# r9y9/deepvoice3_pytorch

Measured on NVIDIA H100. Metric: mel-frames/sec training step (B=16,T_mel=800), higher is better.
Workload: dtype f32 via split 16-bit pairs (fp16 pairs forward, bf16 pairs for gradients; 3 wgmma passes per product, fp32 accumulate)

## Files before the change

deepvoice3_pytorch_b200/csrc/tc_gemm.cu:

```cuda
#include "tc_common.cuh"
#include "../../include/dv3b200.h"

namespace dv3 {

using namespace tc;

constexpr int TC_CONV_THREADS = 512;
constexpr int TC_PRODUCER_REGS = 24;
constexpr int TC_CONSUMER_REGS = 176;
constexpr int TC_EPILOGUE_REGS = 136;
static_assert(TC_PRODUCER_REGS <= 65536 / TC_CONV_THREADS && TC_CONSUMER_REGS >= 65536 / TC_CONV_THREADS &&
              TC_EPILOGUE_REGS >= 65536 / TC_CONV_THREADS, "setmaxnreg direction of each warpgroup");
static_assert(128 * TC_PRODUCER_REGS + 256 * TC_CONSUMER_REGS + 128 * TC_EPILOGUE_REGS <= 65536, "register file");
constexpr int MAX_TAPS_TC = 8;
constexpr int SMEM_LIMIT = 232448;
constexpr int RING_RESERVE = 32768;

template <int STAGE_BYTES, int TILE_COLS, int RESERVE>
struct RingCfg {
    static constexpr int STAGE = STAGE_BYTES;
    static constexpr int NCOLS = TILE_COLS;
    static constexpr int ACC_PITCH = NCOLS + 1;
    static constexpr int ACC_TILE = 128 * ACC_PITCH * 4;
    static constexpr int STAGES_RAW = (SMEM_LIMIT - 2048 - RESERVE - ACC_TILE) / STAGE;
    static constexpr int STAGES = STAGES_RAW > 6 ? 6 : STAGES_RAW;
    static constexpr int SMEM = STAGES * STAGE + ACC_TILE + 1024 + 512;
};

enum { TC_GATED = 0, TC_CONV = 1 };

struct TcMaps { CUtensorMap a[2]; CUtensorMap b[2]; };

struct TcParams {
    int T;
    int Nc;
    int rows_per_tap;
    int k, kb_n;
    int tap_off[MAX_TAPS_TC];
    const float* bias; const float* spk; const float* res;
    float* y; float* save_a; float* save_s;
    int gate_mode, residual;
    float* out; const float* e1; const float* e2; float alpha; int addmode, relu;
    float p_drop; const unsigned long long* seed_ptr; uint32_t salt;
    float gmain;
    int operand_bf16;
};

template <int BK> struct SwizzleOf;
template <> struct SwizzleOf<64> { static constexpr uint32_t layout = WG_SW128, sbo = 1024; };
template <> struct SwizzleOf<32> { static constexpr uint32_t layout = WG_SW64, sbo = 512; };

template <int BK>
__device__ __forceinline__ uint64_t make_desc(uint32_t saddr) {
    return make_wgmma_desc(saddr, 16, SwizzleOf<BK>::sbo, SwizzleOf<BK>::layout);
}

template <int NBOX, int BK, int BR, int NPL = 2>
using TcCfg = RingCfg<NPL * (128 + NBOX * BR) * BK * 2, BR * NBOX, RING_RESERVE>;
static_assert(TcCfg<2, 32, 64>::STAGES == 4, "gated forward: 4-stage ring");
static_assert(TcCfg<1, 32, 128>::STAGES == 4, "128-column conv: 4-stage ring");
static_assert(TcCfg<1, 64, 64>::STAGES == 3, "64-column conv at BK = 64: 3-stage ring");
static_assert(TcCfg<1, 32, 64>::STAGES == 6, "64-column conv at BK = 32: 6-stage ring");
static_assert(TcCfg<2, 64, 64, 1>::STAGES == 4, "single-pass gated forward: 4-stage ring");
static_assert(TcCfg<1, 64, 128, 1>::STAGES == 4, "single-pass 128-column conv at BK = 64: 4-stage ring");
static_assert(TcCfg<1, 32, 128, 1>::STAGES == 6, "single-pass 128-column conv at BK = 32: 6-stage ring");
static_assert(TcCfg<1, 64, 64, 1>::STAGES == 6, "single-pass 64-column conv at BK = 64: 6-stage ring");
static_assert(TcCfg<1, 32, 64, 1>::STAGES == 6, "single-pass 64-column conv at BK = 32: 6-stage ring");

template <int BR>
__device__ __forceinline__ void epilogue_gated(const TcParams& p, const float* arow, uint64_t* acc_empty, int a_row0,
                                               int a_z, int b_row0) {
    const int t = a_row0 + (threadIdx.x & 127), b = a_z, C = p.Nc;
    const bool tv = t < p.T;
    const float* __restrict__ bias = p.bias;
    const float* __restrict__ res = p.res;
    const float* __restrict__ spk = p.spk;
    float* __restrict__ yo = p.y;
    float* __restrict__ ao = p.save_a;
    float* __restrict__ so = p.save_s;
    const bool need_res = (p.gate_mode != 0) || p.residual;
    const size_t base = ((size_t)b * C + b_row0) * p.T + (tv ? t : 0);
#pragma unroll
    for (int c32 = 0; c32 < BR; c32 += 32) {
        float rr[32], sp[32];
        if (tv) {
            const size_t cb = base + (size_t)c32 * p.T;
#pragma unroll
            for (int i = 0; i < 32; ++i) rr[i] = need_res ? __ldg(&res[cb + (size_t)i * p.T]) : 0.f;
            if (spk) {
#pragma unroll
                for (int i = 0; i < 32; ++i) sp[i] = __ldg(&spk[cb + (size_t)i * p.T]);
            }
#pragma unroll
            for (int i = 0; i < 32; ++i) {
                const int c = b_row0 + c32 + i;
                const size_t idx = cb + (size_t)i * p.T;
                float va = arow[c32 + i];
                if (spk) va += sp[i];
                const float a = va + __ldg(&bias[c]);
                const float s = sigmoidf_(arow[BR + c32 + i] + __ldg(&bias[C + c]));
                float y;
                if (p.gate_mode == 0) {
                    y = a * s;
                    if (p.residual) y = (y + rr[i]) * 0.70710678118654752f;
                } else {
                    y = s * a + (1.f - s) * rr[i];
                }
                yo[idx] = y;
                if (ao) ao[idx] = a;
                if (so) so[idx] = s;
            }
        }
        if (c32 + 32 == BR) mbar_arrive(acc_empty);
    }
}

template <int NCOLS>
__device__ __forceinline__ void epilogue_conv(const TcParams& p, const float* arow, uint64_t* acc_empty, int a_row0,
                                              int a_z, int b_row0) {
    const int t = a_row0 + (threadIdx.x & 127), b = a_z;
    const bool tv = t < p.T;
    const DropCfg drop = make_drop(p.p_drop, p.seed_ptr, p.salt);
    const float* __restrict__ bias = p.bias;
    const float* __restrict__ e1 = p.e1;
    const float* __restrict__ e2 = p.e2;
    float* __restrict__ out = p.out;
#pragma unroll 1
    for (int c32 = 0; c32 < NCOLS; c32 += 32) {
        float v[32], x2[32];
        const int n0 = b_row0 + c32;
        const size_t cb = ((size_t)b * p.Nc + n0) * p.T + (tv ? t : 0);
        if (tv) {
#pragma unroll
            for (int i = 0; i < 32; ++i) {
                const bool ok = n0 + i < p.Nc;
                v[i] = (p.addmode != 0 && ok) ? __ldg(&e1[cb + (size_t)i * p.T]) : 0.f;
                x2[i] = (p.addmode == 2 && ok) ? __ldg(&e2[cb + (size_t)i * p.T]) : 0.f;
            }
#pragma unroll
            for (int i = 0; i < 32; ++i) {
                const int n = n0 + i;
                if (n < p.Nc) {
                    const size_t idx = cb + (size_t)i * p.T;
                    float g = arow[c32 + i] * drop_scale(drop, (uint32_t)idx);
                    if (bias) g += __ldg(&bias[n]);
                    if (p.addmode == 1) g += p.alpha * v[i];
                    else if (p.addmode == 2) g += v[i] * (1.f - x2[i]);
                    if (p.relu) g = fmaxf(g, 0.f);
                    out[idx] = g;
                }
            }
        }
        if (c32 + 32 == NCOLS) mbar_arrive(acc_empty);
    }
}

template <class Cfg, int NPL, class Decode, class Load, class Mma, class Gmain, class Epilogue>
__device__ __forceinline__ void tc_pipeline(const TcMaps& maps, int num_units, Decode decode, Load load, Mma mma,
                                            Gmain gmain, Epilogue epilogue) {
    static_assert(NPL == 1 || NPL == 2, "one or two operand planes");
    static_assert(Cfg::NCOLS <= 128, "main + cross accumulators must fit in the registers of a consumer thread");
    static_assert(Cfg::STAGES >= 2, "pipeline needs at least two stages");
    constexpr int STAGE = Cfg::STAGE, STAGES = Cfg::STAGES;
    constexpr int NR = Cfg::NCOLS / 2;
    pdl_trigger();
    extern __shared__ uint8_t smem_raw[];
    uint8_t* smem = reinterpret_cast<uint8_t*>((reinterpret_cast<uintptr_t>(smem_raw) + 1023) & ~(uintptr_t)1023);
    float* acc_tile = reinterpret_cast<float*>(smem + STAGES * STAGE);
    uint64_t* full = reinterpret_cast<uint64_t*>(smem + STAGES * STAGE + Cfg::ACC_TILE);
    uint64_t* empty = full + STAGES;
    uint64_t* acc_full = empty + STAGES;
    uint64_t* acc_empty = acc_full + 1;
    const int warp = threadIdx.x >> 5, lane = threadIdx.x & 31;

    if (threadIdx.x == 0) {
#pragma unroll
        for (int pl = 0; pl < NPL; ++pl) prefetch_tmap(&maps.a[pl]);
#pragma unroll
        for (int pl = 0; pl < NPL; ++pl) prefetch_tmap(&maps.b[pl]);
        for (int s = 0; s < STAGES; ++s) { mbar_init(&full[s], 1); mbar_init(&empty[s], 2); }
        mbar_init(acc_full, 256);
        mbar_init(acc_empty, 128);
        fence_barrier_init();
    }
    __syncthreads();
    pdl_wait();

    if (warp >= 12) {
        setmaxnreg_inc<TC_EPILOGUE_REGS>();
        int n = 0;
        for (int u = blockIdx.x; u < num_units; u += gridDim.x, ++n) {
            const auto w = decode(u);
            mbar_wait(acc_full, n & 1);
            epilogue(w, acc_tile, acc_empty);
        }
    } else if (warp >= 8) {
        setmaxnreg_dec<TC_PRODUCER_REGS>();
        if (warp == 8 && lane == 0) {
            int it = 0;
            for (int u = blockIdx.x; u < num_units; u += gridDim.x) {
                const auto w = decode(u);
                for (int kit = 0; kit < w.n_iters; ++kit, ++it) {
                    const int s = it % STAGES, ph = (it / STAGES) & 1;
                    mbar_wait(&empty[s], ph ^ 1);
                    mbar_arrive_expect_tx(&full[s], STAGE);
                    load(w, kit, smem + s * STAGE, &full[s]);
                }
            }
        }
    } else {
        setmaxnreg_inc<TC_CONSUMER_REGS>();
        const int wg = warp >> 2, wq = warp & 3;
        float acc[NR], xacc[NPL == 2 ? NR : 1];
        int it = 0, n = 0;
        for (int u = blockIdx.x; u < num_units; u += gridDim.x, ++n) {
            const auto w = decode(u);
#pragma unroll
            for (int i = 0; i < NR; ++i) {
                acc[i] = 0.f;
                if constexpr (NPL == 2) xacc[i] = 0.f;
            }
            for (int kit = 0; kit < w.n_iters; ++kit, ++it) {
                const int s = it % STAGES, ph = (it / STAGES) & 1;
                mbar_wait(&full[s], ph);
                wgmma_fence();
                mma(smem + s * STAGE, wg, acc, xacc);
                wgmma_commit();
                wgmma_wait<1>();
                if (kit > 0 && (threadIdx.x & 127) == 0) mbar_arrive(&empty[(it - 1) % STAGES]);
            }
            wgmma_wait<0>();
            if (w.n_iters > 0 && (threadIdx.x & 127) == 0) mbar_arrive(&empty[(it - 1) % STAGES]);
            const float gm = gmain(w);
            mbar_wait(acc_empty, (n & 1) ^ 1);
#pragma unroll
            for (int i = 0; i < NR; ++i) {
                float* dst = &acc_tile[(64 * wg + frag_row(i, wq, lane)) * Cfg::ACC_PITCH + frag_col(i, lane)];
                if constexpr (NPL == 2) *dst = fmaf(xacc[i], LO_INV, acc[i] * gm);
                else *dst = acc[i] * gm;
            }
            mbar_arrive(acc_full);
        }
    }
}

template <int MODE, int NBOX, int BR, int BK, bool BF16, int NPL>
__global__ void __launch_bounds__(TC_CONV_THREADS, 1)
tc_conv_kernel(const __grid_constant__ TcMaps maps, const __grid_constant__ TcParams p, int tiles_x, int tiles_y,
               int num_tiles) {
    using Cfg = TcCfg<NBOX, BK, BR, NPL>;
    constexpr int NCOLS = Cfg::NCOLS;
    constexpr int TILE = 128 * BK * 2, TILE_B = BR * BK * 2;
    constexpr int B_OFF = NPL * TILE;
    constexpr int A_HALF = 64 * BK * 2;
    const int n_iters = p.k * p.kb_n;

    struct Tile { int a_row0, a_z, b_row0, b_row1, n_iters; };
    auto decode = [&](int tile) {
        Tile w;
        const int ty = tile % tiles_y, r = tile / tiles_y;
        w.a_z = r / tiles_x;
        w.a_row0 = (r % tiles_x) * 128;
        if (MODE == TC_GATED) { w.b_row0 = ty * BR; w.b_row1 = p.Nc + ty * BR; }
        else { w.b_row0 = ty * BR * NBOX; w.b_row1 = w.b_row0 + BR; }
        w.n_iters = n_iters;
        return w;
    };
    auto load = [&](const Tile& w, int kit, uint8_t* st, uint64_t* bar) {
        const int j = kit / p.kb_n, kb = kit - j * p.kb_n;
        const int ax = kb * BK, ay = w.a_row0 + p.tap_off[j];
        const int by0 = j * p.rows_per_tap + w.b_row0, by1 = j * p.rows_per_tap + w.b_row1;
#pragma unroll
        for (int pl = 0; pl < NPL; ++pl) {
            tma_load_3d(st + pl * TILE, &maps.a[pl], bar, ax, ay, w.a_z);
            uint8_t* bdst = st + B_OFF + pl * NBOX * TILE_B;
            tma_load_3d(bdst, &maps.b[pl], bar, ax, by0, 0);
            if (NBOX == 2) tma_load_3d(bdst + TILE_B, &maps.b[pl], bar, ax, by1, 0);
        }
    };
    auto mma = [&](const uint8_t* st, int wg, float* acc, float* xacc) {
        const uint32_t sa = smem_u32(st) + wg * A_HALF, sb = smem_u32(st + B_OFF);
#pragma unroll
        for (int kk = 0; kk < BK / 16; ++kk) {
            const uint32_t ko = kk * 32;
            const uint64_t a0 = make_desc<BK>(sa + ko), b0 = make_desc<BK>(sb + ko);
            wgmma_mma<NCOLS, 0, 0>(BF16, acc, a0, b0, 1);
            if constexpr (NPL == 2) {
                const uint64_t a1 = make_desc<BK>(sa + TILE + ko), b1 = make_desc<BK>(sb + NBOX * TILE_B + ko);
                wgmma_mma<NCOLS, 0, 0>(BF16, xacc, a0, b1, 1);
                wgmma_mma<NCOLS, 0, 0>(BF16, xacc, a1, b0, 1);
            }
        }
    };
    auto gmain = [&](const Tile&) { return p.gmain; };
    auto epilogue = [&](const Tile& w, const float* acc_tile, uint64_t* acc_empty) {
        const float* arow = acc_tile + (threadIdx.x & 127) * Cfg::ACC_PITCH;
        if (MODE == TC_GATED) epilogue_gated<BR>(p, arow, acc_empty, w.a_row0, w.a_z, w.b_row0);
        else epilogue_conv<NCOLS>(p, arow, acc_empty, w.a_row0, w.a_z, w.b_row0);
    };
    tc_pipeline<Cfg, NPL>(maps, num_tiles, decode, load, mma, gmain, epilogue);
}

struct TcMnParams {
    int T, B, Mw, Nw, k;
    int tap_off[MAX_TAPS_TC];
    int nsplit, batches_per_split, kb_n;
    int tiles_n, tiles_m, num_units;
    float* dw; long long split_stride;
    int msplit; long long s_m, s_mh, s_n, s_j;
    float gcoef;
};

constexpr int WG_BOX = 64 * 32 * 2;
template <int NPL>
using WgCfg = RingCfg<NPL * 4 * WG_BOX, 128, 0>;
static_assert(WgCfg<2>::STAGES == 5, "two-plane weight gradient: 5-stage ring");
static_assert(WgCfg<1>::STAGES == 6, "single-pass weight gradient: 6-stage ring");
static_assert(WgCfg<2>::SMEM <= SMEM_LIMIT && WgCfg<1>::SMEM <= SMEM_LIMIT, "weight gradient shared memory");

template <int NPL>
__global__ void __launch_bounds__(TC_CONV_THREADS, 1)
tc_wgrad_mn_kernel(const __grid_constant__ TcMaps maps, const __grid_constant__ TcMnParams p) {
    using Cfg = WgCfg<NPL>;
    constexpr int A_PL = 2 * WG_BOX, B_PL = 2 * WG_BOX;
    constexpr uint32_t LBO = 4096, SBO = 1024;

    struct Unit { int m0, n0, j, s, b_beg, n_iters; };
    auto decode = [&](int u) {
        Unit w;
        w.n0 = (u % p.tiles_n) * 128;
        int r = u / p.tiles_n;
        w.m0 = (r % p.tiles_m) * 128;
        r /= p.tiles_m;
        w.j = r % p.k;
        w.s = r / p.k;
        w.b_beg = w.s * p.batches_per_split;
        const int b_end = min(p.B, w.b_beg + p.batches_per_split);
        w.n_iters = (b_end > w.b_beg ? b_end - w.b_beg : 0) * p.kb_n;
        return w;
    };
    auto load = [&](const Unit& w, int kit, uint8_t* st, uint64_t* bar) {
        const int bi = kit / p.kb_n, tc_ = kit - bi * p.kb_n;
        const int b = w.b_beg + bi, t0 = tc_ * 32;
#pragma unroll
        for (int pl = 0; pl < NPL; ++pl) {
#pragma unroll
            for (int h = 0; h < 2; ++h)
                tma_load_3d(st + pl * A_PL + h * WG_BOX, &maps.a[pl], bar, w.m0 + h * 64, t0, b);
#pragma unroll
            for (int q = 0; q < 2; ++q)
                tma_load_3d(st + NPL * A_PL + pl * B_PL + q * WG_BOX, &maps.b[pl], bar, w.n0 + q * 64,
                            t0 + p.tap_off[w.j], b);
        }
    };
    auto mma = [&](const uint8_t* st, int wg, float* acc, float* xacc) {
        const uint32_t sa = smem_u32(st);
#pragma unroll
        for (int kk = 0; kk < 2; ++kk) {
            const uint32_t ko = kk * 16 * 128;
            const uint64_t a0 = make_wgmma_desc(sa + wg * WG_BOX + ko, LBO, SBO, WG_SW128);
            const uint64_t b0 = make_wgmma_desc(sa + NPL * A_PL + ko, LBO, SBO, WG_SW128);
            wgmma_mma<128, 1, 1>(true, acc, a0, b0, 1);
            if constexpr (NPL == 2) {
                const uint64_t a1 = make_wgmma_desc(sa + A_PL + wg * WG_BOX + ko, LBO, SBO, WG_SW128);
                const uint64_t b1 = make_wgmma_desc(sa + 2 * A_PL + B_PL + ko, LBO, SBO, WG_SW128);
                wgmma_mma<128, 1, 1>(true, xacc, a0, b1, 1);
                wgmma_mma<128, 1, 1>(true, xacc, a1, b0, 1);
            }
        }
    };
    auto gmain = [&](const Unit& w) { return 1.f + p.gcoef * (float)(2 * w.n_iters); };
    auto epilogue = [&](const Unit& w, const float* acc_tile, uint64_t* acc_empty) {
        const int r = threadIdx.x & 127;
        float* __restrict__ out = p.dw + (size_t)w.s * p.split_stride + (size_t)w.j * p.s_j;
        const int rows = min(128, p.Mw - w.m0), cols = min(128, p.Nw - w.n0);
        if (p.s_n == 1) {
            if (r < cols) {
                float* __restrict__ o = out + w.n0 + r;
#pragma unroll 4
                for (int i = 0; i < rows; ++i) {
                    const int m = w.m0 + i;
                    o[(size_t)(m % p.msplit) * p.s_m + (size_t)(m / p.msplit) * p.s_mh] = acc_tile[i * Cfg::ACC_PITCH + r];
                }
            }
        } else if (r < rows) {
            const int m = w.m0 + r;
            float* __restrict__ o = out + (size_t)(m % p.msplit) * p.s_m + (size_t)(m / p.msplit) * p.s_mh +
                                    (size_t)w.n0 * p.s_n;
            const float* arow = acc_tile + r * Cfg::ACC_PITCH;
#pragma unroll 4
            for (int c = 0; c < cols; ++c) o[(size_t)c * p.s_n] = arow[c];
        }
        mbar_arrive(acc_empty);
    };
    tc_pipeline<Cfg, NPL>(maps, p.num_units, decode, load, mma, gmain, epilogue);
}

typedef CUresult (*EncodeTiledFn)(CUtensorMap*, CUtensorMapDataType, cuuint32_t, void*, const cuuint64_t*,
                                  const cuuint64_t*, const cuuint32_t*, const cuuint32_t*, CUtensorMapInterleave,
                                  CUtensorMapSwizzle, CUtensorMapL2promotion, CUtensorMapFloatOOBfill);

static EncodeTiledFn encode_fn() {
    static const EncodeTiledFn fn = [] {
        void* f = nullptr;
        cudaDriverEntryPointQueryResult qres;
        cudaError_t e = cudaGetDriverEntryPoint("cuTensorMapEncodeTiled", &f, cudaEnableDefault, &qres);
        return (e == cudaSuccess) ? (EncodeTiledFn)f : (EncodeTiledFn) nullptr;
    }();
    return fn;
}

int encode_tmap_bf16_3d(CUtensorMap* map, const void* base, uint64_t d0, uint64_t d1, uint64_t d2,
                        uint64_t stride1_bytes, uint64_t stride2_bytes, uint32_t box0, uint32_t box1) {
    const EncodeTiledFn enc = encode_fn();
    if (!enc) { set_error("cuTensorMapEncodeTiled entry point unavailable"); return 1; }
    cuuint64_t dims[3] = {d0, d1, d2};
    cuuint64_t strides[2] = {stride1_bytes, stride2_bytes};
    cuuint32_t box[3] = {box0, box1, 1};
    cuuint32_t estr[3] = {1, 1, 1};
    const CUtensorMapSwizzle sw = box0 * 2 == 128 ? CU_TENSOR_MAP_SWIZZLE_128B : CU_TENSOR_MAP_SWIZZLE_64B;
    CUresult r = enc(map, CU_TENSOR_MAP_DATA_TYPE_BFLOAT16, 3, const_cast<void*>(base), dims, strides, box, estr,
                     CU_TENSOR_MAP_INTERLEAVE_NONE, sw, CU_TENSOR_MAP_L2_PROMOTION_L2_256B,
                     CU_TENSOR_MAP_FLOAT_OOB_FILL_NONE);
    if (r != CUDA_SUCCESS) {
        set_error("cuTensorMapEncodeTiled failed (%d): dims=(%llu,%llu,%llu) strides=(%llu,%llu) box=(%u,%u)", (int)r,
                  (unsigned long long)d0, (unsigned long long)d1, (unsigned long long)d2,
                  (unsigned long long)stride1_bytes, (unsigned long long)stride2_bytes, box0, box1);
        return 1;
    }
    return 0;
}

template <typename K>
static int ensure_smem(K kern, int bytes, const char* what) {
    cudaError_t e = cudaFuncSetAttribute(kern, cudaFuncAttributeMaxDynamicSharedMemorySize, bytes);
    if (e != cudaSuccess) { set_error("%s: cannot set %d B dynamic smem: %s", what, bytes, cudaGetErrorString(e)); return 1; }
    return 0;
}

template <class Cfg, auto kern, typename... Args>
static int launch_persistent(int units, cudaStream_t st, const char* what, const Args&... args) {
    static const int configured = ensure_smem(kern, Cfg::SMEM, what);
    if (configured) return 1;
    const int sms = config().sms, grid = units < sms ? units : sms;
    cudaError_t e = launch_k(kern, dim3(grid), dim3(TC_CONV_THREADS), (size_t)Cfg::SMEM, st, args...);
    if (e != cudaSuccess) { set_error("%s: launch failed: %s", what, cudaGetErrorString(e)); return 1; }
    return check_launch(what);
}

template <int MODE, int NBOX, int BR, int BK, bool BF16, int NPL>
static int launch_conv_fmt(const TcMaps& maps, const TcParams& p, int tiles_x, int tiles_y, int batch, cudaStream_t st,
                           const char* what) {
    const int num_tiles = tiles_x * tiles_y * batch;
    return launch_persistent<TcCfg<NBOX, BK, BR, NPL>, tc_conv_kernel<MODE, NBOX, BR, BK, BF16, NPL>>(
        num_tiles, st, what, maps, p, tiles_x, tiles_y, num_tiles);
}

template <int MODE, int NBOX, int BR, int BK, int NPL = 2>
static int launch_conv(const TcMaps& maps, const TcParams& p, int tiles_x, int tiles_y, int batch, cudaStream_t st,
                       const char* what) {
    if (p.operand_bf16)
        return launch_conv_fmt<MODE, NBOX, BR, BK, true, NPL>(maps, p, tiles_x, tiles_y, batch, st, what);
    return launch_conv_fmt<MODE, NBOX, BR, BK, false, NPL>(maps, p, tiles_x, tiles_y, batch, st, what);
}

static void fill_taps_tc(int* tap_off, int k, int dilation, int causal, bool transpose) {
    const int padl = causal ? (k - 1) * dilation : (k - 1) / 2 * dilation;
    for (int j = 0; j < MAX_TAPS_TC; ++j)
        tap_off[j] = j < k ? (transpose ? (padl - j * dilation) : (j * dilation - padl)) : 0;
}

static inline const void* plane(const void* base, int pl, long long plane_elems) {
    return (const char*)base + (size_t)pl * plane_elems * 2;
}

}

using namespace dv3;

extern "C" {

int dv3_tc_supported(int B, int C, int T, int k) {
    return (C % 128 == 0) && T >= 1 && k >= 1 && k <= MAX_TAPS_TC && B >= 1 && B <= 65535;
}
int dv3_tc_conv_supported(int B, int Cin, int Cout, int T, int k) {
    return T >= 1 && k >= 1 && k <= MAX_TAPS_TC && B >= 1 && B <= 65535 && (k == 1 || Cout % 128 == 0) && Cin >= 8 &&
           Cout >= 1;
}

int dv3_tc_convblock_fwd(const void* xd, const void* w, int npl, const float* bias, const float* spk,
                         const float* res, float* y, float* save_a, float* save_s, int B, int C, int T, int k,
                         int dilation, int causal, int mode, int residual, const void* fuse, void* stream) {
    DV3_REQUIRE(dv3_tc_supported(B, C, T, k), "tc_convblock_fwd: unsupported shape B=%d C=%d T=%d k=%d", B, C, T, k);
    DV3_REQUIRE(npl == 1 || npl == 2, "tc_convblock_fwd: npl must be 1 or 2");
    DV3_REQUIRE(fuse == nullptr, "tc_convblock_fwd: fuse must be NULL");
    TcMaps maps;
    const int t_tiles = (T + 127) / 128;
    const int BK = npl == 2 ? 32 : 64;
    for (int pl = 0; pl < npl; ++pl) {
        if (encode_tmap_bf16_3d(&maps.a[pl], plane(xd, pl, (long long)B * T * C), C, T, B, (uint64_t)C * 2,
                                (uint64_t)T * C * 2, BK, 128)) return 1;
        if (encode_tmap_bf16_3d(&maps.b[pl], plane(w, pl, (long long)k * 2 * C * C), C, (uint64_t)k * 2 * C, 1,
                                (uint64_t)C * 2, (uint64_t)k * 2 * C * C * 2, BK, 64)) return 1;
    }
    TcParams p = {};
    p.T = T; p.Nc = C; p.rows_per_tap = 2 * C; p.k = k; p.kb_n = C / BK;
    fill_taps_tc(p.tap_off, k, dilation, causal, false);
    p.bias = bias; p.spk = spk; p.res = res; p.y = y; p.save_a = save_a; p.save_s = save_s;
    p.gate_mode = mode; p.residual = residual;
    p.gmain = 1.f + config().tc_gamma * (float)(p.k * p.kb_n * (BK / 16));
    cudaStream_t st = (cudaStream_t)stream;
    if (npl == 1)
        return launch_conv_fmt<TC_GATED, 2, 64, 64, false, 1>(maps, p, t_tiles, C / 64, B, st, "tc_convblock_fwd");
    return launch_conv_fmt<TC_GATED, 2, 64, 32, false, 2>(maps, p, t_tiles, C / 64, B, st, "tc_convblock_fwd");
}

int dv3_tc_conv(const void* a, const void* w, int npl, float* out, int B, int Kc, int Nc, int T, int k, int dilation,
                int causal, int transpose_taps, const float* bias, int relu, float p_drop,
                const unsigned long long* seed_ptr, unsigned salt, int addmode, const float* e1, const float* e2,
                float alpha, const void* fuse, void* stream) {
    DV3_REQUIRE(k >= 1 && k <= MAX_TAPS_TC && (k == 1 || Nc % 128 == 0) && B <= 65535,
                "tc_conv: unsupported shape B=%d Kc=%d Nc=%d T=%d k=%d", B, Kc, Nc, T, k);
    DV3_REQUIRE(npl == 1 || npl == 2, "tc_conv: npl must be 1 or 2");
    DV3_REQUIRE(fuse == nullptr, "tc_conv: fuse must be NULL");
    const int Kp = (Kc + 7) / 8 * 8;
    const int t_tiles = (T + 127) / 128;
    cudaStream_t st = (cudaStream_t)stream;
    const long long tiles128 = (long long)t_tiles * ((Nc + 127) / 128) * B;
    const bool narrow = Nc > 64 && (k == 1 || Nc % 64 == 0) && tiles128 < 100;
    const bool k64 = Kc % 64 == 0;
    const int bk = ((narrow || npl == 1) && k64) ? 64 : 32, br = narrow ? 64 : 128;
    TcMaps maps;
    for (int pl = 0; pl < npl; ++pl) {
        if (encode_tmap_bf16_3d(&maps.a[pl], plane(a, pl, (long long)B * T * Kp), Kc, T, B, (uint64_t)Kp * 2,
                                (uint64_t)T * Kp * 2, bk, 128)) return 1;
        if (encode_tmap_bf16_3d(&maps.b[pl], plane(w, pl, (long long)k * Nc * Kp), Kc, (uint64_t)k * Nc, 1,
                                (uint64_t)Kp * 2, (uint64_t)k * Nc * Kp * 2, bk, br)) return 1;
    }
    TcParams p = {};
    p.T = T; p.Nc = Nc; p.rows_per_tap = Nc; p.k = k; p.kb_n = (Kc + bk - 1) / bk;
    fill_taps_tc(p.tap_off, k, dilation, causal, transpose_taps != 0);
    p.out = out; p.bias = bias; p.relu = relu; p.e1 = e1; p.e2 = e2; p.alpha = alpha; p.addmode = addmode;
    p.p_drop = p_drop; p.seed_ptr = seed_ptr; p.salt = salt;
    p.gmain = 1.f + config().tc_gamma * (float)(p.k * p.kb_n * (bk / 16));
    p.operand_bf16 = transpose_taps ? 1 : 0;
    const int tiles_y = (Nc + br - 1) / br;
    if (npl == 1) {
        if (narrow) {
            if (k64) return launch_conv<TC_CONV, 1, 64, 64, 1>(maps, p, t_tiles, tiles_y, B, st, "tc_conv(64)");
            return launch_conv<TC_CONV, 1, 64, 32, 1>(maps, p, t_tiles, tiles_y, B, st, "tc_conv(64,bk32)");
        }
        if (k64) return launch_conv<TC_CONV, 1, 128, 64, 1>(maps, p, t_tiles, tiles_y, B, st, "tc_conv(128,bk64)");
        return launch_conv<TC_CONV, 1, 128, 32, 1>(maps, p, t_tiles, tiles_y, B, st, "tc_conv(128)");
    }
    if (narrow) {
        if (k64) return launch_conv<TC_CONV, 1, 64, 64>(maps, p, t_tiles, tiles_y, B, st, "tc_conv(64)");
        return launch_conv<TC_CONV, 1, 64, 32>(maps, p, t_tiles, tiles_y, B, st, "tc_conv(64,bk32)");
    }
    return launch_conv<TC_CONV, 1, 128, 32>(maps, p, t_tiles, tiles_y, B, st, "tc_conv(128)");
}

constexpr double WG_UNIT_ITERS = 25.0;
constexpr double WG_SLAB_BYTES_PER_ITER = 1.5e6;
int dv3_tc_wgrad_nsplit(int B, int Mw, int Nw, int T, int k) {
    const long long tk = (long long)((Mw + 127) / 128) * ((Nw + 127) / 128) * k;
    const long long kb_n = (T + 31) / 32, sms = config().sms;
    const double slab = (double)Mw * Nw * k * 8.0 / WG_SLAB_BYTES_PER_ITER;
    auto cost = [&](int ns) {
        const long long bps = (B + ns - 1) / ns, U = tk * ns, U_full = tk * (ns - 1), G = U < sms ? U : sms;
        const long long L = bps * kb_n, L_last = (B - (ns - 1) * bps) * kb_n;
        return (double)((U_full + G - 1) / G) * (double)(L - L_last) +
               (double)((U + G - 1) / G) * ((double)L_last + WG_UNIT_ITERS) + ns * slab;
    };
    double best = 0.0;
    for (int bps = B, prev = 0; bps >= 1; --bps) {
        const int ns = (B + bps - 1) / bps;
        if (ns != prev && (prev == 0 || cost(ns) < best)) best = cost(ns);
        prev = ns;
    }
    for (int bps = B, prev = 0; bps >= 1; --bps) {
        const int ns = (B + bps - 1) / bps;
        if (ns != prev && cost(ns) <= 1.03 * best) return ns;
        prev = ns;
    }
    return 1;
}

int dv3_tc_wgrad_mn_npl(const void* dy, const void* xd, int npl, float* dw_partials, long long split_stride, int B,
                        int Mw, int Nw, int T, int k, int dilation, int causal, int msplit, long long s_m,
                        long long s_mh, long long s_n, long long s_j, void* stream) {
    DV3_REQUIRE(k >= 1 && k <= MAX_TAPS_TC && B <= 65535, "tc_wgrad_mn: unsupported shape k=%d", k);
    DV3_REQUIRE(npl == 1 || npl == 2, "tc_wgrad_mn: npl must be 1 or 2");
    const int Mp = (Mw + 7) / 8 * 8, Np = (Nw + 7) / 8 * 8;
    TcMaps maps;
    for (int pl = 0; pl < npl; ++pl) {
        if (encode_tmap_bf16_3d(&maps.a[pl], plane(dy, pl, (long long)B * T * Mp), Mw, T, B, (uint64_t)Mp * 2,
                                (uint64_t)T * Mp * 2, 64, 32)) return 1;
        if (encode_tmap_bf16_3d(&maps.b[pl], plane(xd, pl, (long long)B * T * Np), Nw, T, B, (uint64_t)Np * 2,
                                (uint64_t)T * Np * 2, 64, 32)) return 1;
    }
    TcMnParams p = {};
    p.T = T; p.B = B; p.Mw = Mw; p.Nw = Nw; p.k = k; p.kb_n = (T + 31) / 32;
    fill_taps_tc(p.tap_off, k, dilation, causal, false);
    p.nsplit = dv3_tc_wgrad_nsplit(B, Mw, Nw, T, k);
    p.batches_per_split = (B + p.nsplit - 1) / p.nsplit;
    p.tiles_n = (Nw + 127) / 128; p.tiles_m = (Mw + 127) / 128;
    const long long units = (long long)p.tiles_n * p.tiles_m * k * p.nsplit;
    DV3_REQUIRE(units < (1ll << 31), "tc_wgrad_mn: %lld work units", units);
    p.num_units = (int)units;
    p.dw = dw_partials; p.split_stride = split_stride;
    p.msplit = msplit; p.s_m = s_m; p.s_mh = s_mh; p.s_n = s_n; p.s_j = s_j;
    p.gcoef = config().tc_gamma;
    cudaStream_t st = (cudaStream_t)stream;
    if (npl == 1)
        return launch_persistent<WgCfg<1>, tc_wgrad_mn_kernel<1>>(p.num_units, st, "tc_wgrad_mn", maps, p);
    return launch_persistent<WgCfg<2>, tc_wgrad_mn_kernel<2>>(p.num_units, st, "tc_wgrad_mn", maps, p);
}

int dv3_tc_wgrad_mn(const void* dy, const void* xd, float* dw_partials, long long split_stride, int B, int Mw,
                    int Nw, int T, int k, int dilation, int causal, int msplit, long long s_m, long long s_mh,
                    long long s_n, long long s_j, void* stream) {
    return dv3_tc_wgrad_mn_npl(dy, xd, 2, dw_partials, split_stride, B, Mw, Nw, T, k, dilation, causal, msplit, s_m,
                               s_mh, s_n, s_j, stream);
}

}
```

include/dv3b200.h:

```cpp
#ifndef DV3B200_H
#define DV3B200_H

#ifdef __cplusplus
extern "C" {
#endif

const char* dv3_last_error(void);
int dv3_abi_version(void);
long long dv3_launch_count(void);

int dv3_weightnorm_fwd(const float* v, const float* g, float* inv_norm, float* scale, float* out1,
                       float* out2, int R, int X, int k, long long s1r, long long s1x, long long s1j,
                       long long s2r, long long s2x, long long s2j, void* stream);
int dv3_weightnorm_bwd(float* dw_partials, long long split_stride, int nsplit, int tap_major, const float* v,
                       const float* g, const float* inv_norm, float* dv, float* dg, int R, int X, int k,
                       int accumulate, void* stream);

int dv3_convblock_fwd(const float* x, const float* w_f, const float* bias, const float* spk, float* y,
                      float* save_a, float* save_s, int B, int C, int T, int k, int dilation, int causal,
                      int mode, int residual, float p_drop, const unsigned long long* seed_ptr,
                      unsigned salt, void* stream);
int dv3_convblock_gate_bwd(const float* dy, const float* a, const float* s, const float* x, float* dab,
                           float* dbias, int B, int C, int T, int mode, int residual, void* stream);

// ... 78 lines not shown
                         void* stream);

int dv3_resample_out_len(int n_samples, int up, int down);
int dv3_resample_poly_batched(const void* wav, int wav_int16, const int* lengths, int pitch_in, float* out,
                              int pitch_out, int nclips, const double* bank, int up, int down, int ntaps,
                              int pre_remove, void* stream);
int dv3_resample_segments_batched(const void* wav, int wav_int16, int pitch_in, const int* seg, int nclips, float* out,
                                  int pitch_out, const double* bank, int up, int down, int ntaps, int pre_remove,
                                  void* stream);
int dv3_trim_bounds_batched(const void* wav, int wav_int16, const int* lengths, const int* offsets, int pitch,
                            int nclips, const double* top_db, int* bounds, void* stream);

int dv3_spec_to_amp(const float* spec_norm, float* amp, long long n, float min_level_db, float ref_level_db,
                    float power, void* stream);
int dv3_lws_nofuture(const float* mag, float* spec, const float* weights, int nframes, int init_iters, void* stream);
int dv3_lws_iterate(const float* mag, const float* spec_in, float* spec_out, const float* weights, int nframes,
                    void* stream);
int dv3_lws_nofuture_batched(const float* mag, float* spec, const float* weights, const int* nframes, int max_frames,
                             int nclips, int init_iters, void* stream);
int dv3_lws_iterate_batched(const float* mag, const float* spec_in, float* spec_out, const float* weights,
                            const int* nframes, int max_frames, int nclips, void* stream);
int dv3_deemphasis(const float* x, float* y, int nclips, int n_samples, long long stride, float coef, void* stream);

int dv3_stft_num_frames_geom(int n_samples, int n_fft, int hop);
int dv3_stft_mel_geom(const void* wav, int wav_int16, const int* lengths, const float* peak, float rescaling_max,
                      const float* table, const float* mel_basis, const int* mel_start, const int* mel_len,
                      float* linear, float* mel, int nclips, int max_len, int T_lin, int lead, int downsample_step,
                      int n_mels, int n_fft, int hop, float preemph, float min_level_db, float ref_level_db,
                      void* stream);
int dv3_stft_complex_geom(const float* wav, const int* n_samples, long long wav_pitch, const float* mag, float* spec,
                          const int* nframes, int max_frames, int nclips, const float* table, int n_fft, int hop,
                          void* stream);
int dv3_istft_geom(const float* spec, float* wav, const int* n_samples, long long wav_pitch, const int* nframes,
                   int max_frames, int nclips, const float* table, int n_fft, int hop, void* stream);
int dv3_stft_complex_momentum_geom(const float* wav, const int* n_samples, long long wav_pitch, const float* mag,
                                   float* prev, float* spec, const int* nframes, int max_frames, int nclips,
                                   float beta, const float* table, int n_fft, int hop, void* stream);
int dv3_lws_nofuture_geom(const float* mag, float* spec, const float* weights, const int* nframes, int max_frames,
                          int nclips, int init_iters, int n_fft, int hop, void* stream);
int dv3_lws_iterate_geom(const float* mag, const float* spec_in, float* spec_out, const float* weights,
                         const int* nframes, int max_frames, int nclips, int n_fft, int hop, void* stream);

int dv3_tc_supported(int B, int C, int T, int k);
int dv3_tc_conv_supported(int B, int Cin, int Cout, int T, int k);
int dv3_tc_split_input(const float* x, void* btc, int npl, void* bct, int B, int C, int T, int k, int dilation,
                       int causal, float p_drop, const unsigned long long* seed_ptr, unsigned salt, void* stream);
int dv3_tc_gate_bwd_split(const float* dy, const float* a, const float* s, const float* x, void* btc, void* bct,
                          float* dbias, int B, int C, int T, int mode, int residual, void* stream);
int dv3_tc_grad_split(const float* dy, const float* y, void* btc, void* bct, float* dbias, int B, int C, int T,
                      int relu, void* stream);
int dv3_tc_split_input_ext(const float* x, void* btc, int npl, void* bct, int B, int C, int T, float p_drop,
                           const unsigned long long* seed_ptr, unsigned salt, const long long* tlen, int tmult,
                           void* stream);
int dv3_tc_gate_bwd_split_ext(const float* dy, const float* a, const float* s, const float* x, void* btc, void* bct,
                              float* dbias, int B, int C, int T, int mode, int residual, const long long* tlen,
                              int tmult, void* stream);
int dv3_tc_grad_split_ext(const float* dy, const float* y, void* btc, void* bct, float* dbias, int B, int C, int T,
                          int relu, const long long* tlen, int tmult, void* stream);
int dv3_tc_gate_bwd_split_npl(const float* dy, const float* a, const float* s, const float* x, void* btc, int npl,
                              void* bct, float* dbias, int B, int C, int T, int mode, int residual,
                              const long long* tlen, int tmult, void* stream);
int dv3_tc_grad_split_npl(const float* dy, const float* y, void* btc, int npl, void* bct, float* dbias, int B, int C,
                          int T, int relu, const long long* tlen, int tmult, void* stream);
int dv3_tc_weightnorm_fwd(const float* v, const float* g, float* inv_norm, float* scale, void* wfwd, int npl,
                          void* wbwd, int Cout, int Cin, int k, void* stream);
int dv3_tc_weightnorm_convt_fwd(const float* v, const float* g, float* inv_norm, float* scale, void* wfwd, int npl,
                                void* wbwd, int Cin, int Cout, void* stream);
typedef struct Dv3WnEntry {
    const float* v; const float* g; float* inv_norm; float* scale;
    void* wfwd; void* wbwd;
    float* partials; float* dv; float* dg;
    long long split_stride;
    int Cout, Cin, k, nsplit;
    int blk_norm, blk_pack, blk_bwd, pack_gx;
} Dv3WnEntry;
int dv3_tc_weightnorm_fwd_batched(const Dv3WnEntry* table_dev, int n, int norm_blocks, int pack_blocks,
                                  void* stream);
int dv3_tc_weightnorm_fwd_batched_npl(const Dv3WnEntry* table_dev, int n, int norm_blocks, int pack_blocks, int npl,
                                      void* stream);
int dv3_weightnorm_bwd_batched(const Dv3WnEntry* table_dev, int n, int bwd_blocks, int accumulate, void* stream);
int dv3_tc_convblock_fwd(const void* xd, const void* w, int npl, const float* bias, const float* spk,
                         const float* res, float* y, float* save_a, float* save_s, int B, int C, int T, int k,
                         int dilation, int causal, int mode, int residual, const void* fuse, void* stream);
int dv3_tc_conv(const void* a, const void* w, int npl, float* out, int B, int Kc, int Nc, int T, int k, int dilation,
                int causal, int transpose_taps, const float* bias, int relu, float p_drop,
                const unsigned long long* seed_ptr, unsigned salt, int addmode, const float* e1, const float* e2,
                float alpha, const void* fuse, void* stream);
int dv3_tc_wgrad_nsplit(int B, int Mw, int Nw, int T, int k);
int dv3_tc_wgrad_mn(const void* dy, const void* xd, float* dw_partials, long long split_stride, int B, int Mw,
                    int Nw, int T, int k, int dilation, int causal, int msplit, long long s_m, long long s_mh,
                    long long s_n, long long s_j, void* stream);
int dv3_tc_wgrad_mn_npl(const void* dy, const void* xd, int npl, float* dw_partials, long long split_stride, int B,
                        int Mw, int Nw, int T, int k, int dilation, int causal, int msplit, long long s_m,
                        long long s_mh, long long s_n, long long s_j, void* stream);

int dv3_spec_loss(const float* y_hat, const float* y, const long long* lengths, float* grad, float* loss, int B,
                  int T, int D, int r, float masked_loss_weight, float binary_divergence_weight, int priority_bin,
                  float priority_weight, void* stream);
int dv3_aux_loss(const float* done_hat, const float* done, float* d_done, long long n_done, const float* attn,
                 float* d_attn, const long long* in_len, const long long* dec_len, int A, int B, int Td, int Ts,
                 float sigma, int use_attn, float* loss, void* stream);
int dv3_spec_loss_ext(const float* y_hat, const float* y, const long long* lengths, const long long* t_log,
                      float* grad, float* loss, int B, int T, int D, int r, float masked_loss_weight,
                      float binary_divergence_weight, int priority_bin, float priority_weight, void* stream);
int dv3_aux_loss_ext(const float* done_hat, const float* done, float* d_done, const float* attn, float* d_attn,
                     const long long* in_len, const long long* dec_len, const long long* ext, int A, int B, int Td,
                     int Ts, float sigma, int use_attn, float* loss, void* stream);
enum { DV3_TERM_MEL_L1 = 0, DV3_TERM_MEL_BD = 1, DV3_TERM_LIN_L1 = 2, DV3_TERM_LIN_BD = 3, DV3_TERM_DONE = 4,
       DV3_TERM_ATTN = 5, DV3_TERM_COUNT = 6 };
int dv3_spec_loss_terms(const float* y_hat, const float* y, const long long* lengths, const long long* t_log,
                        float* grad, float* loss, float* terms, int B, int T, int D, int r, float masked_loss_weight,
                        float binary_divergence_weight, int priority_bin, float priority_weight, void* stream);
int dv3_aux_loss_terms(const float* done_hat, const float* done, float* d_done, long long n_done, const float* attn,
                       float* d_attn, const long long* in_len, const long long* dec_len, const long long* ext, int A,
                       int B, int Td, int Ts, float sigma, int use_attn, float* loss, float* terms, void* stream);

int dv3_loss_det_scratch_floats(void);
int dv3_spec_loss_det(const float* y_hat, const float* y, const long long* lengths, const long long* t_log,
                      float* grad, float* loss, float* terms, float* scratch, int B, int T, int D, int r,
                      float masked_loss_weight, float binary_divergence_weight, int priority_bin,
                      float priority_weight, void* stream);
int dv3_aux_loss_det(const float* done_hat, const float* done, float* d_done, long long n_done, const float* attn,
                     float* d_attn, const long long* in_len, const long long* dec_len, const long long* ext, int A,
                     int B, int Td, int Ts, float sigma, int use_attn, float* loss, float* terms, float* scratch,
                     void* stream);
long long dv3_bias_det_scratch_floats(int B, int nch, int T, int tiled);
int dv3_convblock_gate_bwd_det(const float* dy, const float* a, const float* s, const float* x, float* dab,
                               float* dbias, float* scratch, long long scratch_floats, int B, int C, int T, int mode,
                               int residual, void* stream);
int dv3_bias_act_bwd_det(const float* dy, const float* y, float* dyr, float* dbias, float* scratch,
                         long long scratch_floats, int B, int C, int T, int relu, void* stream);
int dv3_tc_gate_bwd_split_det(const float* dy, const float* a, const float* s, const float* x, void* btc, int npl,
                              float* dbias, float* scratch, long long scratch_floats, int B, int C, int T, int mode,
                              int residual, const long long* tlen, int tmult, void* stream);
int dv3_tc_grad_split_det(const float* dy, const float* y, void* btc, int npl, float* dbias, float* scratch,
                          long long scratch_floats, int B, int C, int T, int relu, const long long* tlen, int tmult,
                          void* stream);
int dv3_embedding_bwd_det(const long long* ids, const float* dy, float* dtable, int N, int D, int V,
                          long long padding_idx, void* stream);
int dv3_sinusoid_bwd_det(const long long* pos, const float* table, const float* w, int nw, const float* dy,
                         float* dtable, float* dw, int B, int T, int D, int P, void* stream);

typedef struct Dv3IncStep {
    const float* x; long long x_ld, x_t;
    const float* add; long long add_ld, add_t;
    float* ring;
    const float* w; const float* bias;
    const float* spk; long long spk_ld;
    const float* res1; long long res1_ld, res1_t;
    const float* res2; long long res2_ld, res2_t;
    float* y; long long y_ld, y_t;
    float* y2; long long y2_ld, y2_t;
    const float* yadd; long long yadd_ld, yadd_t;
    const int* t_ptr;
    int B, Cin, Cout, k, dilation;
    int mode;
    int act;
    int vec4;
    int y2_mode;
} Dv3IncStep;
int dv3_inc_conv_step(const Dv3IncStep* step, void* stream);
typedef struct Dv3IncAttn {
    const float* q; long long q_ld;
    const float* keys; const float* values;
    float* ctx; long long ctx_ld;
    float* align; long long align_ld, align_t;
// ... 76 lines not shown
```

Baseline: 1.543 million.

## Load a shared activation window once for all three conv taps

For two-plane convolutions with three taps whose offsets fit in a 192-row span, each pipeline stage now loads one widened activation window plus the weight boxes of all three taps. The MMA reads each tap's A operand at a row offset inside that window, so the per-tap reloads of overlapping activation rows go away and the k-loop runs kb_n iterations instead of k*kb_n. The cost is bigger 48 KB stages, and this path forces BK=32 and 64-column tiles even where a 128-column or BK=64 config was chosen before. It also relies on row offsets that are multiples of 8 keeping the swizzled descriptors valid.

```diff
diff --git a/deepvoice3_pytorch_b200/csrc/tc_gemm.cu b/deepvoice3_pytorch_b200/csrc/tc_gemm.cu
--- a/deepvoice3_pytorch_b200/csrc/tc_gemm.cu
+++ b/deepvoice3_pytorch_b200/csrc/tc_gemm.cu
@@ -37,6 +37,7 @@
     int rows_per_tap;
     int k, kb_n;
     int tap_off[MAX_TAPS_TC];
+    int win_off, win_tx;
     const float* bias; const float* spk; const float* res;
     float* y; float* save_a; float* save_s;
     int gate_mode, residual;
@@ -66,6 +67,11 @@
 static_assert(TcCfg<1, 32, 128, 1>::STAGES == 6, "single-pass 128-column conv at BK = 32: 6-stage ring");
 static_assert(TcCfg<1, 64, 64, 1>::STAGES == 6, "single-pass 64-column conv at BK = 64: 6-stage ring");
 static_assert(TcCfg<1, 32, 64, 1>::STAGES == 6, "single-pass 64-column conv at BK = 32: 6-stage ring");
+
+constexpr int WIN_TAPS = 3, WIN_ROWS = 192;
+using WinCfg = RingCfg<2 * (WIN_ROWS + WIN_TAPS * 64) * 32 * 2, 64, 0>;
+static_assert(WinCfg::STAGES == 4, "window 64-column conv: 4 stages of 48 KB");
+static_assert(WIN_ROWS * 32 * 2 % 1024 == 0, "window planes keep the B boxes on swizzle-atom boundaries");
 
 template <int BR>
 __device__ __forceinline__ void epilogue_gated(const TcParams& p, const float* arow, uint64_t* acc_empty, int a_row0,
@@ -156,8 +162,8 @@
 }
 
 template <class Cfg, int NPL, class Decode, class Load, class Mma, class Gmain, class Epilogue>
-__device__ __forceinline__ void tc_pipeline(const TcMaps& maps, int num_units, Decode decode, Load load, Mma mma,
-                                            Gmain gmain, Epilogue epilogue) {
+__device__ __forceinline__ void tc_pipeline(const TcMaps& maps, int num_units, uint32_t stage_tx, Decode decode,
+                                            Load load, Mma mma, Gmain gmain, Epilogue epilogue) {
     static_assert(NPL == 1 || NPL == 2, "one or two operand planes");
     static_assert(Cfg::NCOLS <= 128, "main + cross accumulators must fit in the registers of a consumer thread");
     static_assert(Cfg::STAGES >= 2, "pipeline needs at least two stages");
@@ -203,7 +209,7 @@
                 for (int kit = 0; kit < w.n_iters; ++kit, ++it) {
                     const int s = it % STAGES, ph = (it / STAGES) & 1;
                     mbar_wait(&empty[s], ph ^ 1);
-                    mbar_arrive_expect_tx(&full[s], STAGE);
+                    mbar_arrive_expect_tx(&full[s], stage_tx);
                     load(w, kit, smem + s * STAGE, &full[s]);
                 }
             }
@@ -244,16 +250,19 @@
     }
 }
 
-template <int MODE, int NBOX, int BR, int BK, bool BF16, int NPL>
+template <int MODE, int NBOX, int BR, int BK, bool BF16, bool WIN, int NPL>
 __global__ void __launch_bounds__(TC_CONV_THREADS, 1)
 tc_conv_kernel(const __grid_constant__ TcMaps maps, const __grid_constant__ TcParams p, int tiles_x, int tiles_y,
                int num_tiles) {
-    using Cfg = TcCfg<NBOX, BK, BR, NPL>;
+    static_assert(!WIN || (MODE == TC_CONV && NBOX == 1 && BR == 64 && BK == 32 && NPL == 2), "window stages");
+    using Cfg = std::conditional_t<WIN, WinCfg, TcCfg<NBOX, BK, BR, NPL>>;
     constexpr int NCOLS = Cfg::NCOLS;
-    constexpr int TILE = 128 * BK * 2, TILE_B = BR * BK * 2;
-    constexpr int B_OFF = NPL * TILE;
-    constexpr int A_HALF = 64 * BK * 2;
-    const int n_iters = p.k * p.kb_n;
+    constexpr int TAPS = WIN ? WIN_TAPS : 1;
+    constexpr int A_ROWS = WIN ? WIN_ROWS : 128;
+    constexpr int TILE = A_ROWS * BK * 2, TILE_B = BR * BK * 2;
+    constexpr int B_OFF = NPL * TILE, B_PL = TAPS * NBOX * TILE_B;
+    constexpr int ROW = BK * 2;
+    const int n_iters = WIN ? p.kb_n : p.k * p.kb_n;
 
     struct Tile { int a_row0, a_z, b_row0, b_row1, n_iters; };
     auto decode = [&](int tile) {
@@ -267,28 +276,40 @@
         return w;
     };
     auto load = [&](const Tile& w, int kit, uint8_t* st, uint64_t* bar) {
-        const int j = kit / p.kb_n, kb = kit - j * p.kb_n;
-        const int ax = kb * BK, ay = w.a_row0 + p.tap_off[j];
-        const int by0 = j * p.rows_per_tap + w.b_row0, by1 = j * p.rows_per_tap + w.b_row1;
+        const int j0 = WIN ? 0 : kit / p.kb_n, kb = kit - j0 * p.kb_n;
+        const int ax = kb * BK, ay = w.a_row0 + (WIN ? p.win_off : p.tap_off[j0]);
 #pragma unroll
         for (int pl = 0; pl < NPL; ++pl) {
             tma_load_3d(st + pl * TILE, &maps.a[pl], bar, ax, ay, w.a_z);
-            uint8_t* bdst = st + B_OFF + pl * NBOX * TILE_B;
-            tma_load_3d(bdst, &maps.b[pl], bar, ax, by0, 0);
-            if (NBOX == 2) tma_load_3d(bdst + TILE_B, &maps.b[pl], bar, ax, by1, 0);
+#pragma unroll
+            for (int t = 0; t < TAPS; ++t) {
+                const int j = j0 + t;
+                uint8_t* bdst = st + B_OFF + pl * B_PL + t * NBOX * TILE_B;
+                tma_load_3d(bdst, &maps.b[pl], bar, ax, j * p.rows_per_tap + w.b_row0, 0);
+                if (NBOX == 2) tma_load_3d(bdst + TILE_B, &maps.b[pl], bar, ax, j * p.rows_per_tap + w.b_row1, 0);
+            }
         }
     };
     auto mma = [&](const uint8_t* st, int wg, float* acc, float* xacc) {
-        const uint32_t sa = smem_u32(st) + wg * A_HALF, sb = smem_u32(st + B_OFF);
-#pragma unroll
-        for (int kk = 0; kk < BK / 16; ++kk) {
-            const uint32_t ko = kk * 32;
-            const uint64_t a0 = make_desc<BK>(sa + ko), b0 = make_desc<BK>(sb + ko);
-            wgmma_mma<NCOLS, 0, 0>(BF16, acc, a0, b0, 1);
-            if constexpr (NPL == 2) {
-                const uint64_t a1 = make_desc<BK>(sa + TILE + ko), b1 = make_desc<BK>(sb + NBOX * TILE_B + ko);
-                wgmma_mma<NCOLS, 0, 0>(BF16, xacc, a0, b1, 1);
-                wgmma_mma<NCOLS, 0, 0>(BF16, xacc, a1, b0, 1);
+#ifdef DV3_TC_LOADS_ONLY
+        return;
+#endif
+        const uint32_t s0 = smem_u32(st), sb = smem_u32(st + B_OFF);
+#pragma unroll
+        for (int t = 0; t < TAPS; ++t) {
+            const uint32_t sa = s0 + (WIN ? 64 * wg + p.tap_off[t] - p.win_off : 64 * wg) * ROW;
+            const uint32_t st_b = sb + t * NBOX * TILE_B;
+#pragma unroll
+            for (int kk = 0; kk < BK / 16; ++kk) {
+                const uint32_t ko = kk * 32;
+                const uint64_t a0 = make_desc<BK>(sa + ko), b0 = make_desc<BK>(st_b + ko);
+                wgmma_mma<NCOLS, 0, 0>(BF16, acc, a0, b0, 1);
+                if constexpr (NPL == 2) {
+                    const uint64_t a1 = make_desc<BK>(sa + TILE + ko);
+                    const uint64_t b1 = make_desc<BK>(st_b + B_PL + ko);
+                    wgmma_mma<NCOLS, 0, 0>(BF16, xacc, a0, b1, 1);
+                    wgmma_mma<NCOLS, 0, 0>(BF16, xacc, a1, b0, 1);
+                }
             }
         }
     };
@@ -298,7 +319,8 @@
         if (MODE == TC_GATED) epilogue_gated<BR>(p, arow, acc_empty, w.a_row0, w.a_z, w.b_row0);
         else epilogue_conv<NCOLS>(p, arow, acc_empty, w.a_row0, w.a_z, w.b_row0);
     };
-    tc_pipeline<Cfg, NPL>(maps, num_tiles, decode, load, mma, gmain, epilogue);
+    tc_pipeline<Cfg, NPL>(maps, num_tiles, WIN ? (uint32_t)p.win_tx : (uint32_t)Cfg::STAGE, decode, load, mma, gmain,
+                          epilogue);
 }
 
 struct TcMnParams {
@@ -393,7 +415,7 @@
         }
         mbar_arrive(acc_empty);
     };
-    tc_pipeline<Cfg, NPL>(maps, p.num_units, decode, load, mma, gmain, epilogue);
+    tc_pipeline<Cfg, NPL>(maps, p.num_units, Cfg::STAGE, decode, load, mma, gmain, epilogue);
 }
 
 typedef CUresult (*EncodeTiledFn)(CUtensorMap*, CUtensorMapDataType, cuuint32_t, void*, const cuuint64_t*,
@@ -448,20 +470,21 @@
     return check_launch(what);
 }
 
-template <int MODE, int NBOX, int BR, int BK, bool BF16, int NPL>
+template <int MODE, int NBOX, int BR, int BK, bool BF16, int NPL, bool WIN = false>
 static int launch_conv_fmt(const TcMaps& maps, const TcParams& p, int tiles_x, int tiles_y, int batch, cudaStream_t st,
                            const char* what) {
+    using Cfg = std::conditional_t<WIN, WinCfg, TcCfg<NBOX, BK, BR, NPL>>;
     const int num_tiles = tiles_x * tiles_y * batch;
-    return launch_persistent<TcCfg<NBOX, BK, BR, NPL>, tc_conv_kernel<MODE, NBOX, BR, BK, BF16, NPL>>(
-        num_tiles, st, what, maps, p, tiles_x, tiles_y, num_tiles);
-}
-
-template <int MODE, int NBOX, int BR, int BK, int NPL = 2>
+    return launch_persistent<Cfg, tc_conv_kernel<MODE, NBOX, BR, BK, BF16, WIN, NPL>>(num_tiles, st, what, maps, p,
+                                                                                      tiles_x, tiles_y, num_tiles);
+}
+
+template <int MODE, int NBOX, int BR, int BK, int NPL = 2, bool WIN = false>
 static int launch_conv(const TcMaps& maps, const TcParams& p, int tiles_x, int tiles_y, int batch, cudaStream_t st,
                        const char* what) {
     if (p.operand_bf16)
-        return launch_conv_fmt<MODE, NBOX, BR, BK, true, NPL>(maps, p, tiles_x, tiles_y, batch, st, what);
-    return launch_conv_fmt<MODE, NBOX, BR, BK, false, NPL>(maps, p, tiles_x, tiles_y, batch, st, what);
+        return launch_conv_fmt<MODE, NBOX, BR, BK, true, NPL, WIN>(maps, p, tiles_x, tiles_y, batch, st, what);
+    return launch_conv_fmt<MODE, NBOX, BR, BK, false, NPL, WIN>(maps, p, tiles_x, tiles_y, batch, st, what);
 }
 
 static void fill_taps_tc(int* tap_off, int k, int dilation, int causal, bool transpose) {
@@ -470,6 +493,17 @@
         tap_off[j] = j < k ? (transpose ? (padl - j * dilation) : (j * dilation - padl)) : 0;
 }
 
+static int window_rows(TcParams& p, int npl) {
+    if (npl != 2 || p.k != WIN_TAPS) return 0;
+    int lo = p.tap_off[0], hi = p.tap_off[0];
+    for (int j = 1; j < p.k; ++j) { lo = p.tap_off[j] < lo ? p.tap_off[j] : lo; hi = p.tap_off[j] > hi ? p.tap_off[j] : hi; }
+    const int rows = (128 + hi - lo + 7) / 8 * 8;
+    if (rows > WIN_ROWS) return 0;
+    p.win_off = lo;
+    p.win_tx = 2 * (rows + WIN_TAPS * 64) * 32 * 2;
+    return rows;
+}
+
 static inline const void* plane(const void* base, int pl, long long plane_elems) {
     return (const char*)base + (size_t)pl * plane_elems * 2;
 }
@@ -486,6 +520,14 @@
 int dv3_tc_conv_supported(int B, int Cin, int Cout, int T, int k) {
     return T >= 1 && k >= 1 && k <= MAX_TAPS_TC && B >= 1 && B <= 65535 && (k == 1 || Cout % 128 == 0) && Cin >= 8 &&
            Cout >= 1;
+}
+
+int dv3_tc_window_rows(int npl, int k, int dilation, int causal, int transpose_taps) {
+    if (k < 1 || k > MAX_TAPS_TC) return 0;
+    TcParams p = {};
+    p.k = k;
+    fill_taps_tc(p.tap_off, k, dilation, causal, transpose_taps != 0);
+    return window_rows(p, npl);
 }
 
 int dv3_tc_convblock_fwd(const void* xd, const void* w, int npl, const float* bias, const float* spk,
@@ -497,15 +539,15 @@
     TcMaps maps;
     const int t_tiles = (T + 127) / 128;
     const int BK = npl == 2 ? 32 : 64;
+    TcParams p = {};
+    p.T = T; p.Nc = C; p.rows_per_tap = 2 * C; p.k = k; p.kb_n = C / BK;
+    fill_taps_tc(p.tap_off, k, dilation, causal, false);
     for (int pl = 0; pl < npl; ++pl) {
         if (encode_tmap_bf16_3d(&maps.a[pl], plane(xd, pl, (long long)B * T * C), C, T, B, (uint64_t)C * 2,
                                 (uint64_t)T * C * 2, BK, 128)) return 1;
         if (encode_tmap_bf16_3d(&maps.b[pl], plane(w, pl, (long long)k * 2 * C * C), C, (uint64_t)k * 2 * C, 1,
                                 (uint64_t)C * 2, (uint64_t)k * 2 * C * C * 2, BK, 64)) return 1;
     }
-    TcParams p = {};
-    p.T = T; p.Nc = C; p.rows_per_tap = 2 * C; p.k = k; p.kb_n = C / BK;
-    fill_taps_tc(p.tap_off, k, dilation, causal, false);
     p.bias = bias; p.spk = spk; p.res = res; p.y = y; p.save_a = save_a; p.save_s = save_s;
     p.gate_mode = mode; p.residual = residual;
     p.gmain = 1.f + config().tc_gamma * (float)(p.k * p.kb_n * (BK / 16));
@@ -527,19 +569,22 @@
     const int t_tiles = (T + 127) / 128;
     cudaStream_t st = (cudaStream_t)stream;
     const long long tiles128 = (long long)t_tiles * ((Nc + 127) / 128) * B;
-    const bool narrow = Nc > 64 && (k == 1 || Nc % 64 == 0) && tiles128 < 100;
+    TcParams p = {};
+    p.T = T; p.Nc = Nc; p.rows_per_tap = Nc; p.k = k;
+    fill_taps_tc(p.tap_off, k, dilation, causal, transpose_taps != 0);
+    const int win = window_rows(p, npl);
+    const bool narrow = win || (Nc > 64 && (k == 1 || Nc % 64 == 0) && tiles128 < 100);
     const bool k64 = Kc % 64 == 0;
-    const int bk = ((narrow || npl == 1) && k64) ? 64 : 32, br = narrow ? 64 : 128;
+    const int br = narrow ? 64 : 128;
+    const int bk = (!win && (narrow || npl == 1) && k64) ? 64 : 32;
+    p.kb_n = (Kc + bk - 1) / bk;
     TcMaps maps;
     for (int pl = 0; pl < npl; ++pl) {
         if (encode_tmap_bf16_3d(&maps.a[pl], plane(a, pl, (long long)B * T * Kp), Kc, T, B, (uint64_t)Kp * 2,
-                                (uint64_t)T * Kp * 2, bk, 128)) return 1;
+                                (uint64_t)T * Kp * 2, bk, win ? win : 128)) return 1;
         if (encode_tmap_bf16_3d(&maps.b[pl], plane(w, pl, (long long)k * Nc * Kp), Kc, (uint64_t)k * Nc, 1,
                                 (uint64_t)Kp * 2, (uint64_t)k * Nc * Kp * 2, bk, br)) return 1;
     }
-    TcParams p = {};
-    p.T = T; p.Nc = Nc; p.rows_per_tap = Nc; p.k = k; p.kb_n = (Kc + bk - 1) / bk;
-    fill_taps_tc(p.tap_off, k, dilation, causal, transpose_taps != 0);
     p.out = out; p.bias = bias; p.relu = relu; p.e1 = e1; p.e2 = e2; p.alpha = alpha; p.addmode = addmode;
     p.p_drop = p_drop; p.seed_ptr = seed_ptr; p.salt = salt;
     p.gmain = 1.f + config().tc_gamma * (float)(p.k * p.kb_n * (bk / 16));
@@ -553,6 +598,7 @@
         if (k64) return launch_conv<TC_CONV, 1, 128, 64, 1>(maps, p, t_tiles, tiles_y, B, st, "tc_conv(128,bk64)");
         return launch_conv<TC_CONV, 1, 128, 32, 1>(maps, p, t_tiles, tiles_y, B, st, "tc_conv(128)");
     }
+    if (win) return launch_conv<TC_CONV, 1, 64, 32, 2, true>(maps, p, t_tiles, tiles_y, B, st, "tc_conv(64,window)");
     if (narrow) {
         if (k64) return launch_conv<TC_CONV, 1, 64, 64>(maps, p, t_tiles, tiles_y, B, st, "tc_conv(64)");
         return launch_conv<TC_CONV, 1, 64, 32>(maps, p, t_tiles, tiles_y, B, st, "tc_conv(64,bk32)");
diff --git a/include/dv3b200.h b/include/dv3b200.h
--- a/include/dv3b200.h
+++ b/include/dv3b200.h
@@ -184,6 +184,7 @@
 int dv3_tc_convblock_fwd(const void* xd, const void* w, int npl, const float* bias, const float* spk,
                          const float* res, float* y, float* save_a, float* save_s, int B, int C, int T, int k,
                          int dilation, int causal, int mode, int residual, const void* fuse, void* stream);
+int dv3_tc_window_rows(int npl, int k, int dilation, int causal, int transpose_taps);
 int dv3_tc_conv(const void* a, const void* w, int npl, float* out, int B, int Kc, int Nc, int T, int k, int dilation,
                 int causal, int transpose_taps, const float* bias, int relu, float p_drop,
                 const unsigned long long* seed_ptr, unsigned salt, int addmode, const float* e1, const float* e2,
```

After: 1.586 million, median of 6. 1.03x the previous value.
